# unlikeghost/DeepLearning-MPI

Measured on AMD Instinct MI355X. Metric: images/sec (whole node) ResNet-50 DDP bs=256/GPU, higher is better.
Workload: dtype bf16; 1 GPU; model=resnet50, global_batch=256, image=224, in_channels=3, per_gpu_batch=256, parallelism=dp1, backend=single, device=cuda, optimizer=SGD(momentum=0.9, wd=1e-5), hipgraph=False

## Files before the change

deeplearning_mpi_amd/csrc/binding/conv_bwd.cpp:

```cpp
#include <c10/hip/HIPCachingAllocator.h>

#include <algorithm>
#include <vector>

#include "common.h"
#include "ops.h"

namespace dlmpi_ext {

using dlmpi::ConvArgs;
using dlmpi::ConvPhase;
using dlmpi::DgradStreamArgs;
using dlmpi::make_fastdiv;
using dlmpi::WgradArgs;

c10::optional<at::Tensor> conv2d_dgrad_pro(const at::Tensor& dy, int N, int P, int Q, int K, int lddy, int dyoff,
                                       const at::Tensor& wT, int C, int R, int S, int stride, int pad, int H, int W,
                                       at::Tensor dx, int lddx, int dxoff, const c10::optional<at::Tensor>& res,
                                       int ldres, int resoff, const c10::optional<at::Tensor>& mask, int ldmask,
                                       int maskoff, const c10::optional<at::Tensor>& z, int ldz, int zoff,
                                       const c10::optional<at::Tensor>& z2, int ldz2, int z2off,
                                       const c10::optional<at::Tensor>& mscale,
                                       const c10::optional<at::Tensor>& mshift,
                                       const c10::optional<at::Tensor>& mbits, bool colsum, int pro,
                                       const c10::optional<at::Tensor>& pk0, const c10::optional<at::Tensor>& pk1,
                                       const c10::optional<at::Tensor>& pz, int ldpz, int pzoff,
                                       const c10::optional<at::Tensor>& bias) {
  require_gpu(dy, "dy");
  if (stride > 2) throw std::runtime_error("conv2d_dgrad: stride <= 2 supported");
  if (bias.has_value() && bias->defined() && (bias->scalar_type() != at::kFloat || bias->numel() < C))
    throw std::runtime_error("conv2d_dgrad: bias must be fp32 [C]");
  ConvArgs a{};
  a.f32 = act_f32(dy, "conv2d_dgrad");
  same_type(dy, wT, "conv2d_dgrad wT");
  same_type(dy, dx, "conv2d_dgrad dx");
  same_type(dy, res, "conv2d_dgrad res");
  same_type(dy, mask, "conv2d_dgrad mask");
  same_type(dy, z, "conv2d_dgrad z");
  same_type(dy, z2, "conv2d_dgrad z2");
  a.x = ptr<uint16_t>(dy);
  a.H = P; a.W = Q; a.C = K; a.ldx = lddy; a.xoff = dyoff;
  a.w = ptr<uint16_t>(wT);
  a.ldw = R * S * K;
  a.S = S;
  a.OH = H; a.OW = W;
  a.so = stride; a.sa = 1;
  a.Nimg = N; a.Kout = C;
  fill_epilogue(a, dx, lddx, dxoff, bias, res, ldres, resoff, c10::nullopt, c10::nullopt, false, c10::nullopt);
  a.vec_store = ((lddx % 8) == 0 && (dxoff % 8) == 0) ? 1 : 0;
  a.mask = optr<uint16_t>(mask);
  a.ldmask = ldmask; a.maskoff = maskoff;
  a.z = optr<uint16_t>(z);
  a.ldz = ldz; a.zoff = zoff;
  a.z2 = optr<uint16_t>(z2);
  a.ldz2 = ldz2; a.z2off = z2off;
  a.mscale = optr<float>(mscale);
  a.mshift = optr<float>(mshift);
  a.mbits = optr<uint8_t>(mbits);
  if (a.mbits && (mbits->numel() != (int64_t)N * H * W * (C / 8) || C % 8))
    throw std::runtime_error("conv2d_dgrad: mask bits must be [N*H*W][C/8]");
  a.nstat = a.z2 ? 3 : 2;
  if (a.z && !a.mask && !a.mscale && !a.mbits)
    throw std::runtime_error("conv2d_dgrad: fused BN statistics need the ReLU mask");
  if (a.mscale && (!a.z || !a.mshift)) throw std::runtime_error("conv2d_dgrad: mask from z needs z, scale, shift");
  if ((a.mask || a.mscale || a.mbits) && ((ldmask | maskoff | ldz | zoff | ldz2 | z2off) % 8 != 0 || !a.vec_store))
    throw std::runtime_error("conv2d_dgrad: fused BN tensors must be 8-channel aligned");
  g_ran.dgrad_stream = 0;
  g_ran.conv3 = 0;
  if (R == 1 && S == 1 && K == 8) g_ran.head_dgrad = 0;
  {
    const int mode = a.mscale ? 2 : 0;
    int th, tw, G;
    if (stream3x3_shape(N, H, W, K, C, R, S, stride, pad, pro, a.f32, th, tw, G) && P == H && Q == W && !colsum &&
        !a.mask && !a.mbits && !a.z2 && !a.res && !a.bias && (a.z != nullptr) == (mode == 2) && a.vec_store &&
        a.kvalid == C && (lddy | dyoff) % 8 == 0 && (int64_t)H * W * lddx * 2 < (1ll << 31) &&
        dx.scalar_type() == at::kBFloat16) {
      dlmpi::Conv3StreamArgs c = conv3_args(dy, N, H, W, lddy, dyoff, wT, 1, a.y, lddx, dxoff, th, tw, G);
      c.z = static_cast<const uint16_t*>(a.z);
      c.ldz = ldz; c.zoff = zoff;
      c.mscale = a.mscale; c.mshift = a.mshift;
      c10::optional<at::Tensor> st;
      if (a.z) {
        st = at::empty({(int64_t)G, 2, (int64_t)C}, dy.options().dtype(at::kFloat));
        c.stats = ptr<float>(*st);
      }
      check(dlmpi_conv3x3_stream(&c, mode == 2 ? 2 : 1, cur_stream()), "conv2d_dgrad (stream 3x3)");
      g_ran.conv3 = 1;
      return st;
    }
  }
  {
    const int64_t M = (int64_t)N * H * W;
    const int mode = a.mbits ? 1 : (a.mscale ? 2 : 0);
    int sbm, sbn, G;
    const auto fits = [](int64_t rows, int64_t ld) { return rows * ld < (1ll << 31); };
    if (R == 1 && S == 1 && stride == 1 && pad == 0 && !a.f32 && pro == 0 && !colsum && !a.mask &&
        (a.z != nullptr) == (mode != 0) && a.vec_store && a.kvalid == C && (lddy | dyoff) % 8 == 0 &&
        (!a.res || (ldres | resoff) % 8 == 0) && fits(M, lddy) && fits(M, lddx) && (!a.res || fits(M, ldres)) &&
        (!a.z || fits(M, ldz)) && (!a.z2 || fits(M, ldz2)) && dx.scalar_type() == at::kBFloat16 &&
        dlmpi_dgrad_stream_plan(M, K, C, mode, a.z2 ? 1 : 0, a.res ? 1 : 0, &sbm, &sbn, &G)) {
      DgradStreamArgs sa{};
      sa.x = ptr<uint16_t>(dy);
      sa.ldx = lddy; sa.xoff = dyoff;
      sa.w = ptr<uint16_t>(wT);
      sa.y = reinterpret_cast<uint16_t*>(a.y);
      sa.ldy = lddx; sa.yoff = dxoff;
      sa.y_bytes = (int)std::min<int64_t>(INT32_MAX, (int64_t)dx.numel() * 2);
      sa.M = (int)M; sa.K = K; sa.Kout = C;
      sa.bias = a.bias;
      sa.res = static_cast<const uint16_t*>(a.res);
      sa.ldres = ldres; sa.resoff = resoff;
      sa.z = static_cast<const uint16_t*>(a.z);
      sa.ldz = ldz; sa.zoff = zoff;
      sa.z2 = static_cast<const uint16_t*>(a.z2);
      sa.ldz2 = ldz2; sa.z2off = z2off;
      sa.mbits = a.mbits;
      sa.mscale = a.mscale; sa.mshift = a.mshift;
      sa.G = G; sa.ntiles = C / sbn; sa.mtiles = (int)ceil_div(M, sbm);
      c10::optional<at::Tensor> st;
      if (a.z) {
        st = at::empty({(int64_t)G, (int64_t)a.nstat, (int64_t)C}, dy.options().dtype(at::kFloat));
        sa.stats = ptr<float>(*st);
      }
      check(dlmpi_conv1x1_dgrad_stream(&sa, sbm, sbn, mode, cur_stream()), "conv2d_dgrad (stream 1x1)");
      g_ran.dgrad_stream = 1;
      return st;
    }
  }
  set_kstep(a, K);
  set_prologue(a, pro, pk0, pk1, pz, ldpz, pzoff);
  TileQuery q{(int64_t)N * H * W / (stride * stride), C, (int64_t)R * S * K / (stride * stride), K, R, S, stride, pad,
              H, W, a.f32, pro};
  q.halo_ok = P == H && Q == W;
  q.pipe_ok = g_sw.pipe_dgrad != 0;
  const Tiles t = select_tiles(q);
  int bm = t.bm, bn = t.bn;
  const int pipe = t.pipe;
  const bool halo = t.halo;
  a.ntiles = ceil_div(C, bn);
  a.nphase = stride * stride;
  int tiles = 0;
  for (int ph = 0; ph < stride; ++ph) {
    for (int pw = 0; pw < stride; ++pw) {
      ConvPhase& p = a.ph[ph * stride + pw];
      const int r0 = (ph + pad) % stride, s0 = (pw + pad) % stride;
      p.P = (H - ph + stride - 1) / stride;
      p.Q = (W - pw + stride - 1) / stride;
      p.Tr = r0 < R ? (R - r0 + stride - 1) / stride : 0;
      p.Ts = s0 < S ? (S - s0 + stride - 1) / stride : 0;
      p.dh0 = (ph + pad - r0) / stride; p.dhs = -1;
      p.dw0 = (pw + pad - s0) / stride; p.dws = -1;
      p.wr0 = r0; p.wrs = stride; p.ws0 = s0; p.wss = stride;
      p.oh0 = ph; p.ow0 = pw;
      finish_phase(p, N, K, bm, a.f32);
      p.tile_base = tiles;
      tiles += p.mtiles;
    }
  }
  if (halo) {
    apply_halo(a, N, bm);
    tiles = a.ph[0].mtiles;
// ... 189 lines not shown
  const int bn = a.f32 ? 64 : (w256 ? 256 : 128);
  a.ntiles = ceil_div(a.TC, bn);
  const int tiles = a.mtiles * a.ntiles;
  const int target_blocks = g_sw.wgrad_blocks > 0 ? g_sw.wgrad_blocks : 512;
  const int maxsplit = std::max(1, ceil_div(a.npix, 512));
  int splits = std::max(1, std::min(maxsplit, w256 ? target_blocks / tiles : ceil_div(target_blocks, tiles)));
  int pps = ceil_div(a.npix, splits);
  pps = ceil_div(pps, 64) * 64;
  splits = ceil_div(a.npix, pps);
  a.splits = splits;
  a.pix_per_split = pps;
  a.fdPQ = make_fastdiv((uint32_t)(P * Q));
  a.fdQ = make_fastdiv((uint32_t)Q);
  a.fdC = make_fastdiv((uint32_t)C);
  a.fdS = make_fastdiv((uint32_t)S);
  const int64_t wsz = (int64_t)Ko * a.TC;
  const int G = splits > 1 ? dlmpi_wgrad_reduce_groups(splits, wsz) : 0;
  at::Tensor ws = at::empty({(int64_t)(splits + G) * wsz}, dy.options().dtype(at::kFloat));
  a.ws = ptr<float>(ws);
  check(dlmpi_conv_wgrad(&a, bm, bn, cur_stream()), "conv2d_wgrad");
  wgrad_reduce_or_defer(ws, splits, G, wsz, Ko, R * S, C, Creal, Ko_real, grad);
}

void conv2d_wgrad(const at::Tensor& dy, int lddy, int dyoff, int Ko, const at::Tensor& x, int N, int H, int W, int C,
                  int ldx, int xoff, int R, int S, int stride, int pad, int P, int Q, at::Tensor grad, int Creal,
                  int Ko_real) {
  conv2d_wgrad_pro(dy, lddy, dyoff, Ko, x, N, H, W, C, ldx, xoff, R, S, stride, pad, P, Q, grad, Creal, Ko_real, 0,
                   c10::nullopt, c10::nullopt, 0, 0, 0, c10::nullopt, c10::nullopt);
}

void register_conv_bwd(pybind11::module& m) {
  m.def("conv2d_dgrad", &conv2d_dgrad);
  m.def("conv2d_dgrad_pro", &conv2d_dgrad_pro);
  m.def("conv2d_wgrad", &conv2d_wgrad);
  m.def("conv2d_wgrad_pro", &conv2d_wgrad_pro);
  m.def("set_wgrad_defer", [](bool on) {
    if (!on) wgrad_flush();
    g_wgrad_defer = on;
  });
  m.def("wgrad_flush", &wgrad_flush);
  m.def("wgrad_discard", &wgrad_discard);
  m.def("set_wgrad_batch", [](int n) { g_wgrad_batch = n > 0 && n <= dlmpi::kWgradBatch ? n : dlmpi::kWgradBatch; });
  m.def("set_defer_direct", [](int on) { g_defer_direct = on != 0; });
  m.def("set_wgrad_bypass", [](bool on) { g_wgrad_bypass = on; });
  m.def("wgrad_pending", []() { return (int)g_pending.size(); });
  m.def("wgrad_reduce_launches", []() { return g_reduce_launches; });
  m.def("set_dgrad_stream", [](int mode) { dlmpi_set_dgrad_stream(mode); });
  m.def("set_wgrad_fast", [](int on) { dlmpi_set_wgrad_fast(on); });
  def_int(m, "set_conv_pipe_dgrad", nullptr, &g_sw.pipe_dgrad);
  def_int(m, "set_wgrad3", nullptr, &g_sw.wgrad3);
  def_int(m, nullptr, "wgrad3_last", &g_ran.wgrad3);
  def_int(m, "set_wgrad3_blocks", nullptr, &g_sw.wgrad3_blocks);
  def_int(m, "set_wgrad_blocks", nullptr, &g_sw.wgrad_blocks);
  def_int(m, nullptr, "dgrad_stream_last", &g_ran.dgrad_stream);
  def_int(m, nullptr, "head_dgrad_last", &g_ran.head_dgrad);
}

}
```

deeplearning_mpi_amd/csrc/kernels/conv1x1_dgrad_stream.hip:

```cpp
#include "common.h"

namespace dlmpi {

typedef __attribute__((address_space(3))) void dgs_lds_void;

constexpr int dgs_vmcnt(int n) { return (n & 15) | 0x70 | 0xF00 | ((n >> 4) << 14); }
__device__ __forceinline__ void dgs_barrier() { asm volatile("s_waitcnt lgkmcnt(0)\n\ts_barrier" ::: "memory"); }
__device__ __forceinline__ void dgs_glds(const void* g, char* lds) {
  __builtin_amdgcn_global_load_lds(g, (dgs_lds_void*)lds, 16, 0, 0);
}

template <int BN>
__device__ __forceinline__ int dgs_sw(int r) { return BN == 128 ? (r & 15) : ((r >> 1) & 7); }
template <int BN>
__device__ __forceinline__ int dgs_eoff(int r, int col) {
  return r * (2 * BN) + ((((col >> 3) ^ dgs_sw<BN>(r))) << 4) + ((col & 4) << 1);
}

template <int BM, int BN, int KS, int NW, int WGM, int MASK, bool Z2, bool ADB>
__global__ __launch_bounds__(64 * NW) void conv1x1_dgrad_stream_kernel(const DgradStreamArgs a) {
  constexpr bool Z = MASK != 0;
  static_assert(!Z2 || Z, "z2 needs the fused statistics");
  static_assert(BN == 64 || BN == 128, "tile width");
  constexpr bool RES = !(BN == 64 && BM == 64);
// ... 34 lines not shown
  const int jc = (tid & 7) ^ ((tid >> 3) & 7);
  const int erow = tid / ECH, ej = tid % ECH;
  const char* zp = reinterpret_cast<const char*>(g_zero_page);

  const uint32_t lb = xcd_remap(blockIdx.x, gridDim.x);
  const int nt = lb % a.ntiles, g = lb / a.ntiles;
  const int n0 = nt * BN;
  const bool has_res = RES && a.res != nullptr;

#pragma unroll
  for (int ks = 0; ks < KS; ++ks)
#pragma unroll
    for (int i = 0; i < BL; ++i) {
      const int n = n0 + lrow + RP * i;
      const char* src = (lrow + RP * i < BN && n < a.Kout)
                            ? reinterpret_cast<const char*>(a.w + (int64_t)n * a.K + ks * 64 + 8 * jc) : zp;
      dgs_glds(src, Ws + ks * WROWS * 128 + (RP * i + 8 * wid) * 128);
    }
  auto issue_a = [&](int mt, char* Ab) {
#pragma unroll
    for (int ks = 0; ks < KS; ++ks)
#pragma unroll
      for (int i = 0; i < AL; ++i) {
        const int m = min(mt * BM + lrow + RP * i, a.M - 1);
        dgs_glds(a.x + (uint32_t)(m * a.ldx + a.xoff + ks * 64 + 8 * jc), Ab + ks * BM * 128 + (RP * i + 8 * wid) * 128);
      }
  };
  auto issue_e = [&](int mt, char* Rb, char* Zb, char* Mb) {
#pragma unroll
    for (int i = 0; i < EL; ++i) {
      const int r = erow + EP * i;
      const int m = min(mt * BM + r, a.M - 1);
      const int gj = ej ^ dgs_sw<BN>(r);
      if (has_res)
        dgs_glds(a.res + (uint32_t)(m * a.ldres + a.resoff + n0 + gj * 8), Rb + i * EP * ERB + wid * 1024);
      if constexpr (Z)
        dgs_glds(a.z + (uint32_t)(m * a.ldz + a.zoff + n0 + gj * 8), Zb + i * EP * ERB + wid * 1024);
      if constexpr (Z2)
        dgs_glds(a.z2 + (uint32_t)(m * a.ldz2 + a.z2off + n0 + gj * 8), Zb + (EZ2_OFF - EZ_OFF) + i * EP * ERB + wid * 1024);
    }
    if constexpr (MASK == 1) {
      if (wid < MB_INSTR) {
        const int piece = wid * 64 + lane;
        const int r = piece * MB_PIECE / MBR;
        const int m = min(mt * BM + r, a.M - 1);
        const uint8_t* src = a.mbits + (uint32_t)(m * (a.Kout >> 3) + (n0 >> 3) + (piece * MB_PIECE) % MBR);
        if constexpr (MB_PIECE == 16) __builtin_amdgcn_global_load_lds(src, (dgs_lds_void*)(Mb + wid * 1024), 16, 0, 0);
        else __builtin_amdgcn_global_load_lds(src, (dgs_lds_void*)(Mb + wid * 256), 4, 0, 0);
      }
    }
  };

  const __amdgpu_buffer_rsrc_t yr = __builtin_amdgcn_make_buffer_rsrc(a.y, (short)0, a.y_bytes, 0x00020000);
  f32x4 bq[TN], ms[TN], mh[TN];
#pragma unroll
  for (int ni = 0; ni < TN; ++ni) {
    const int c = n0 + wn * WN + ni * 16 + 4 * fg;
    bq[ni] = a.bias ? *reinterpret_cast<const f32x4*>(a.bias + c) : f32x4{0.f, 0.f, 0.f, 0.f};
    if constexpr (MASK == 2) {
      ms[ni] = *reinterpret_cast<const f32x4*>(a.mscale + c);
      mh[ni] = *reinterpret_cast<const f32x4*>(a.mshift + c);
    }
  }
  float s1[TN][4], s2[TN][4], s3[TN][4];
#pragma unroll
  for (int ni = 0; ni < TN; ++ni)
#pragma unroll
    for (int j = 0; j < 4; ++j) { s1[ni][j] = 0.f; s2[ni][j] = 0.f; s3[ni][j] = 0.f; }
// ... 213 lines not shown
```

deeplearning_mpi_amd/csrc/kernels/dlmpi_kernels.h:

```cpp
#pragma once
#include <hip/hip_runtime_api.h>
#include <stdint.h>

namespace dlmpi {

struct FastDiv {
  uint32_t d, mul, shr;
};
inline FastDiv make_fastdiv(uint32_t d) {
  FastDiv f;
  f.d = d;
  uint32_t l = 0;
  while ((1ull << l) < d) ++l;
  f.mul = (uint32_t)((((1ull << 32) * ((1ull << l) - d)) / d) + 1);
  f.shr = l;
  return f;
}

struct FinArgs {
  int mode;
  double count;
  const float* gamma;
  const float* beta;
  float* running_mean;
// ... 18 lines not shown
  uint16_t* y;
  int ldy, yoff;
  int y_bytes;
  int M, C, Kout;
  const float* bias;
  float* stats;
  int G, ntiles, mtiles;
  int s2, H, W;
  FastDiv fdPQ, fdQ;
  int up2;
  int Cup;
};

struct DgradStreamArgs {
  const uint16_t* x;
  int ldx, xoff;
  const uint16_t* w;
  uint16_t* y;
  int ldy, yoff;
  int y_bytes;
  int M, K, Kout;
  const float* bias;
  const uint16_t* res;
  int ldres, resoff;
  const uint16_t* z;
  int ldz, zoff;
  const uint16_t* z2;
  int ldz2, z2off;
  const uint8_t* mbits;
  const float* mscale;
  const float* mshift;
  float* stats;
  int G, ntiles, mtiles;
};

struct ConvPhase {
  int P, Q;
  int Tr, Ts;
  int dh0, dhs, dw0, dws;
  int wr0, wrs, ws0, wss;
  int oh0, ow0;
  int mtiles;
  int ksteps;
  int tile_base;
  FastDiv fdPQ, fdQ, fdTs;
};

struct ConvArgs {
  const void* x;
  int H, W, C, ldx, xoff;
  const void* w;
  int ldw, S;
  void* y;
  int OH, OW, ldy, yoff;
  int so, sa;
  int out_f32;
  int Nimg, Kout;
  int kvalid;
  int vec_store;
  const float* bias;
  const void* res;
  int ldres, resoff;
  const float* scale;
  const float* shift;
  int relu;
  float* stats;
// ... 267 lines not shown
```

deeplearning_mpi_amd/models/engine.py:

```python
from __future__ import annotations

import contextlib
import os
from typing import NamedTuple, Optional

import torch
import torch.nn as nn

from ..ops.act import Act, Deferred, padc
from ..ops.backend import make_backend
from ..utils.arena import ParamArena
from ..utils.profiler import range as trace_range


@contextlib.contextmanager
def grad_side(be, *tensors):
    side = getattr(be, "side_stream", None)
    if side is None:
        yield
        return
    cur = torch.cuda.current_stream()
    side.wait_stream(cur)
    torch.cuda.set_stream(side)
    try:
# ... 11 lines not shown
def record_on(stream, *objs):
    if _STREAM_HOLD:
        return
    for o in objs:
        if o is None:
            continue
        if isinstance(o, torch.Tensor):
            if o.is_cuda:
                o.record_stream(stream)
        elif isinstance(o, Deferred):
            record_on(stream, *o.bufs())
        elif hasattr(o, "buf") and isinstance(getattr(o, "buf"), torch.Tensor):
            record_on(stream, o.buf)
        elif isinstance(o, (tuple, list)):
            record_on(stream, *o)


_STREAM_HOLD = True

_OUTER_DGRAD = True
_HEAD_DGRAD = True

DEFER_BN_WGRAD = True

DUAL_DGRAD = True
DUAL_MIN_ROWS = 2 * 256 * 28 * 28
DUAL_WGRAD_PRO = True

FUSE_APPLY = True
FUSE_APPLY_MAX_K = 256
FUSE_APPLY_3X3 = True

WGRAD_TAIL_MAIN = True


def img_rows(a, n0: int, n1: int):
    if a is None:
        return None
    if isinstance(a, Deferred):
        return Deferred(a.kind, img_rows(a.src, n0, n1), img_rows(a.z, n0, n1), a.k0, a.k1)
    hw = a.H * a.W
    return Act(a.buf[n0 * hw:n1 * hw], n1 - n0, a.H, a.W, a.C, a.off)


class PendingApply:

    __slots__ = ("y", "z", "scale", "shift", "res", "relu", "mbits", "done")

    def __init__(self, y, z, scale, shift, res, relu, mbits):
        self.y, self.z, self.scale, self.shift, self.res, self.relu, self.mbits = y, z, scale, shift, res, relu, mbits
        self.done = False

    N = property(lambda self: self.y.N)
    H = property(lambda self: self.y.H)
    W = property(lambda self: self.y.W)
    C = property(lambda self: self.y.C)
    device = property(lambda self: self.y.device)

    def resolve(self, be) -> Act:
        if not self.done:
            be.bn_apply(self.z, self.scale, self.shift, self.res, self.relu, self.y, mbits=self.mbits)
            self.done = True
        return self.y


def resolve(be, a):
# ... 171 lines not shown
                if defer_apply == "act":
                    return Deferred.affine(z, scale, shift), ctx
                if defer_apply == "bn":
                    return Deferred.bn(z, scale, shift), ctx
                return z, ctx
            mbits = None
            if save and res is not None and self.relu and self.Kp % 8 == 0:
                mbits = torch.empty(y.rows, self.Kp // 8, dtype=torch.uint8, device=dev)
            if before_res is not None and res is not None:
                before_res()
            ctx = (x, z, y, mean, invstd, scale, shift, res is not None, mbits) if save else None
            if lazy and FUSE_APPLY and out is None:
                return PendingApply(y, z, scale, shift, res, self.relu, mbits), ctx
            be.bn_apply(z, scale, shift, res, self.relu, y, mbits=mbits)
            return y, ctx
        if before_res is not None and res is not None:
            before_res()
        invstd = torch.rsqrt(bn.running_var + bn.eps)
        scale = bn.weight.data * invstd if bn.affine else invstd
        shift = (bn.bias.data if bn.affine else 0.0) - bn.running_mean * scale
        if self.bias is not None:
            shift = shift + self.bias.data * scale
        be.conv_fwd(x, wf, self.Kp, self.R, self.S, self.stride, self.pad, y, res=res, scale=scale.contiguous(),
                    shift=shift.contiguous(), relu=self.relu)
        return y, None

    @staticmethod
    def fuse_spec(ctx, z2=None) -> BwdFuse:
        x, z, y, mean, invstd, scale, shift, has_res, mbits = ctx
        if has_res or z2 is not None:
            return BwdFuse(None if mbits is not None else y, z, z2, mbits=mbits)
        return BwdFuse(None, z, None, scale, shift)

    def bwd(self, be, ctx, dy: Act, need_dx=True, dx_res: Act = None, dyr_out: Act = None, ymask: Act = None,
            use_own_mask=True, pre=None, k2=1, fuse_next=None, colsum=False, before_res=None, dx_out: Act = None):
        ar = self.arena
        bn = self.bn
        dg_in, dg_w, dg_b = None, None, None
        if bn is not None and need_dx and pre is not None and dyr_out is None and self.dual:
            x, z = ctx[0], ctx[1]
            if (z.off == z.C and z.ld == 2 * z.C and dy.off == 0 and dy.ld == z.ld
                    and dy.buf.data_ptr() == z.buf.data_ptr()):
                mean, invstd = ctx[3], ctx[4]
                gam = bn.weight.data if bn.affine else None
                dzd = be.bn_bwd_deferred(dy, z, mean, invstd, gam, ar.grad_flat(bn.weight) if bn.affine else None,
                                         ar.grad_flat(bn.bias) if bn.affine else None, pre=pre, k2=k2)
                with grad_side(be, *bufs(dzd, x)):
                    if bn.affine:
                        ar.ready(bn.weight, bn.bias)
                    if self.bias is not None:
                        ar.ready(self.bias)
                    self._wgrad(be, dzd if (DUAL_WGRAD_PRO and getattr(be, "prologue", False)) else be.materialize(dzd), x)
                    ar.ready(self.conv.weight)
                dg_w, dg_b = be.dual_weights(ar.get_compute(self.h_dg), self.Cp, self.Kp, dzd.k0)
                dg_in = Act(z.buf, z.N, z.H, z.W, 2 * z.C)
                bn = None
        if dg_in is not None:
            x = ctx[0]
        elif bn is not None:
            x, z, y, mean, invstd = ctx[:5]
            if pre is not None:
                mask = None
            else:
                mask = ymask if ymask is not None else (y if (self.relu and use_own_mask) else None)
            gam = bn.weight.data if bn.affine else None
            dgam = ar.grad_flat(bn.weight) if bn.affine else None
            dbet = ar.grad_flat(bn.bias) if bn.affine else None
            defer = not need_dx and DEFER_BN_WGRAD and getattr(be, "prologue", False)
# ... 10 lines not shown
                    if self.bias is not None:
                        ar.ready(self.bias)
                    ar.ready(self.conv.weight)
            else:
                with grad_side(be, *bufs(dz, x)):
                    if bn.affine:
                        ar.ready(bn.weight, bn.bias)
                    if self.bias is not None:
                        ar.ready(self.bias)
                    self._wgrad(be, dz, x)
                    ar.ready(self.conv.weight)
        else:
            x, y = ctx
            assert not self.relu, "ReLU without BN is not used by the engine models"
            dz = dy
            with grad_side(be, *bufs(dz, x)):
                if self.bias is not None:
                    if self.Kp == self.K:
                        be.channel_sum(dz, ar.grad_flat(self.bias))
                    else:
                        tmp = torch.empty(self.Kp, dtype=be.dt, device=dz.device)
                        be.fill_(tmp, 0.0)
                        be.channel_sum(dz, tmp)
                        if getattr(self, "_kidx", None) is None or self._kidx.device != dz.device:
                            self._kidx = torch.arange(self.K, device=dz.device)
                        be.gather_(ar.grad_flat(self.bias), tmp, self._kidx, accumulate=True)
                    ar.ready(self.bias)
                self._wgrad(be, dz, x)
                ar.ready(self.conv.weight)
        if not need_dx:
            return None
        if before_res is not None:
            before_res()
        if dx_out is not None:
            assert (dx_out.N, dx_out.H, dx_out.W, dx_out.C) == (x.N, x.H, x.W, self.Cp), (dx_out, x, self.Cp)
            dx = dx_out
        else:
            dx = Act.empty(x.N, x.H, x.W, self.Cp, be.act_dtype, x.device)
        if dg_in is not None:
            part = be.conv_dgrad(dg_in, dg_w, self.Cp, 1, 1, 1, 0, dx, res=dx_res, fuse=fuse_next, colsum=colsum,
                                 bias=dg_b)
            return (dx, part) if (fuse_next is not None or colsum) else dx
        if (self.K == 1 and self.R == 1 and self.S == 1 and self.stride == 1 and dx_res is None and not colsum
                and fuse_next is not None and fuse_next.scale is not None and fuse_next.z2 is None
                and hasattr(be, "outer_dgrad_bn") and _OUTER_DGRAD):
            part = be.outer_dgrad_bn(be.materialize(dz), ar.get_compute(self.h_dg), self.Kp, dx, fuse_next)
            return dx, part
        if (2 <= self.K <= 4 and self.R == 1 and self.S == 1 and self.stride == 1 and dx_res is None and not colsum
                and fuse_next is not None and fuse_next.scale is not None and fuse_next.z2 is None
                and hasattr(be, "head_dgrad_bn") and _HEAD_DGRAD):
            part = be.head_dgrad_bn(be.materialize(dz), self.K, ar.get_compute(self.h_dg), self.Kp, dx, fuse_next)
            return dx, part
        part = be.conv_dgrad(dz, ar.get_compute(self.h_dg), self.Cp, self.R, self.S, self.stride, self.pad, dx,
                             res=dx_res, fuse=fuse_next, colsum=colsum)
        return (dx, part) if (fuse_next is not None or colsum) else dx


class S2DConvUnit(ConvUnit):

    CS = 4

    def __init__(self, arena: ParamArena, conv, bn=None, relu=True):
        w = conv.weight
        K, Cin, R, S = w.shape
        assert conv.stride == (2, 2) and conv.padding[0] == conv.padding[1] and conv.groups == 1
        assert Cin <= self.CS and conv.dilation == (1, 1)
        self.arena, self.conv, self.bn, self.relu = arena, conv, bn, relu
        self.linear = False
        self.K, self.Cin, self.R0, self.S0, self.pad0 = K, Cin, R, S, conv.padding[0]
        self.R, self.S = (R + 1) // 2, (S + 1) // 2
        self.stride, self.pad = 1, 0
        self.Cp = 4 * self.CS
        self.Kp = padc(K)
        self.bias = conv.bias
        self._bias_pad = None
        self.h_dg = None
        self.h_slots = []
        for vh in (0, 1):
            for vw in (0, 1):
                v = w.data[:, :, vh::2, vw::2]
                self.h_slots.append(arena.add_compute(v, (self.Kp, self.R, self.S, self.CS),
                                                      (K, v.shape[2], v.shape[3], Cin), (0, 2, 3, 1)))
        self.w2 = None
        self._w2idx = None
        arena.post_refresh.append(self._build_w2)
        self._gidx = None

# ... 212 lines not shown
```

deeplearning_mpi_amd/models/resnet.py:

```python
from __future__ import annotations


import torch
import torch.nn as nn
import torch.nn.functional as F

from ..ops.act import Act, padc
from .engine import PendingApply, BwdFuse, ConvUnit, EngineModule, S2DConvUnit, record_on, resolve


def conv3x3(i, o, stride=1):
    return nn.Conv2d(i, o, 3, stride, 1, bias=False)


def conv1x1(i, o, stride=1):
    return nn.Conv2d(i, o, 1, stride, 0, bias=False)


class BasicBlock(nn.Module):
    expansion = 1

    def __init__(self, inplanes, planes, stride=1, downsample=None):
        super().__init__()
        self.conv1 = conv3x3(inplanes, planes, stride)
# ... 85 lines not shown
            ctxs.append(first[1])
        for u in self.u[1 if first is not None else 0:-1]:
            h, c = u.fwd(be, h, train, save=save, lazy=lazy)
            ctxs.append(c)
        join = None
        if br is not None:
            def join():
                main.wait_stream(br)
                record_on(main, idn, cd)
            if not _LATE_JOIN:
                join()
                join = None
        elif self.ud is not None:
            idn, cd = self.ud.fwd(be, x, train, save=save, defer_apply=ds_defer)
        else:
            idn, cd = resolve(be, x), None
        y, c = self.u[-1].fwd(be, h, train, res=idn, save=save, before_res=join, lazy=lazy)
        ctxs.append(c)
        return y, (ctxs, cd)

    def fuse_spec(self, st):
        ctxs, cd = st
        return ConvUnit.fuse_spec(ctxs[-1], z2=cd[1] if cd is not None else None)

    def out_slot(self, st):
        return self.u[-1].dy_slot(st[0][-1])

    def bwd(self, be, st, dy: Act, pre=None, fuse_prev=None, fuse_inner=False, dx_out=None):
        ctxs, cd = st
        slot = lambda k: self.u[k].dy_slot(ctxs[k])
        ylast = ctxs[-1][2]
        n = len(self.u)
        spec = lambda k: ConvUnit.fuse_spec(ctxs[k])
        if pre is not None:
            br = getattr(be, "branch_stream", None) if self.ud is not None else None
            if br is not None:
                main = torch.cuda.current_stream()
                br.wait_stream(main)
                with torch.cuda.stream(br):
                    dres = self.ud.bwd(be, cd, dy, pre=pre, k2=2)
                record_on(br, dy, pre)
            dh, part = self.u[-1].bwd(be, ctxs[-1], dy, pre=pre, k2=1, fuse_next=spec(n - 2), dx_out=slot(n - 2))
            for k in range(n - 2, 0, -1):
                dh, part = self.u[k].bwd(be, ctxs[k], dh, pre=part, fuse_next=spec(k - 1), dx_out=slot(k - 1))
            join = None
            if br is not None:
                def join():
                    main.wait_stream(br)
                    record_on(main, dres)
                if not _LATE_JOIN:
                    join()
                    join = None
            elif self.ud is not None:
                dres = self.ud.bwd(be, cd, dy, pre=pre, k2=2)
            else:
                dres = dy
            return self.u[0].bwd(be, ctxs[0], dh, dx_res=dres, pre=part, fuse_next=fuse_prev, before_res=join,
                                 dx_out=dx_out)
        inner = fuse_inner or any(c[2] is None for c in ctxs[:-1])
        if self.ud is None:
            dyr = Act.empty(dy.N, dy.H, dy.W, dy.C, be.act_dtype, dy.device)
            dh = self.u[-1].bwd(be, ctxs[-1], dy, dyr_out=dyr, fuse_next=spec(n - 2) if inner else None,
                                dx_out=slot(n - 2))
        else:
            dyr = None
            dh = self.u[-1].bwd(be, ctxs[-1], dy, fuse_next=spec(n - 2) if inner else None, dx_out=slot(n - 2))
        part = None
        if inner:
            dh, part = dh
        for k in range(n - 2, 0, -1):
            if inner:
                dh, part = self.u[k].bwd(be, ctxs[k], dh, pre=part, fuse_next=spec(k - 1), dx_out=slot(k - 1))
            else:
                dh = self.u[k].bwd(be, ctxs[k], dh, dx_out=slot(k - 1))
        if self.ud is not None:
            dres = self.ud.bwd(be, cd, dy, ymask=ylast)
        else:
            dres = dyr
        out = self.u[0].bwd(be, ctxs[0], dh, dx_res=dres, pre=part, fuse_next=fuse_prev, dx_out=dx_out)
        return out


class ResNet(EngineModule):
    def __init__(self, block, layers, num_classes=1000, in_channels=3):
        super().__init__()
        self.inplanes = 64
        self.in_channels = in_channels
        self.conv1 = nn.Conv2d(in_channels, 64, kernel_size=7, stride=2, padding=3, bias=False)
        self.bn1 = nn.BatchNorm2d(64)
        self.relu = nn.ReLU(inplace=True)
        self.maxpool = nn.MaxPool2d(kernel_size=3, stride=2, padding=1)
        self.layer1 = self._make_layer(block, 64, layers[0])
        self.layer2 = self._make_layer(block, 128, layers[1], stride=2)
        self.layer3 = self._make_layer(block, 256, layers[2], stride=2)
        self.layer4 = self._make_layer(block, 512, layers[3], stride=2)
        self.avgpool = nn.AdaptiveAvgPool2d((1, 1))
        self.fc = nn.Linear(512 * block.expansion, num_classes)
        for m in self.modules():
            if isinstance(m, nn.Conv2d):
                nn.init.kaiming_normal_(m.weight, mode="fan_out", nonlinearity="relu")
            elif isinstance(m, nn.BatchNorm2d):
                nn.init.constant_(m.weight, 1)
                nn.init.constant_(m.bias, 0)

    def _make_layer(self, block, planes, blocks, stride=1):
        downsample = None
        if stride != 1 or self.inplanes != planes * block.expansion:
            downsample = nn.Sequential(conv1x1(self.inplanes, planes * block.expansion, stride),
                                       nn.BatchNorm2d(planes * block.expansion))
# ... 113 lines not shown
```

deeplearning_mpi_amd/ops/backend.py:

```python
from __future__ import annotations

import os
import weakref
import struct

import torch
import torch.nn.functional as F

from .act import Act, Deferred


_AUX_STREAMS = {}
_BACKENDS = weakref.WeakSet()


def _new_aux_stream(idx, C, role):
    with torch.cuda.device(idx):
        st = torch.cuda.ExternalStream(C.create_stream(), device=torch.device("cuda", idx))
        C.set_aux_stream(st.cuda_stream, role)
    return st


def _aux_stream(device, C, role):
    idx = device.index if device.index is not None else torch.cuda.current_device()
# ... 126 lines not shown
    def conv_fwd_bn_apply(self, xp, w, K, z: Act, bias, stats, count, gamma, beta, rm, rv, momentum, eps, scale,
                          shift, save_mean, save_invstd):
        x, res = xp.z, xp.res
        rs = rh = None
        if isinstance(res, Deferred):
            assert res.kind == "bn", res
            res, rs, rh = res.src, res.k0, res.k1
        y = xp.y
        self.C.conv2d_fwd_bn_apply(x.buf, x.N, x.H, x.W, x.C, x.ld, x.off, w, K, z.buf, z.ld, z.off, bias, stats,
                                   xp.scale, xp.shift, res.buf, res.ld, res.off, rs, rh, y.buf, y.ld, y.off, xp.mbits,
                                   float(count), gamma, beta, rm, rv, float(momentum), float(eps), scale, shift,
                                   save_mean, save_invstd)

    def conv3_pro_ok(self, z: Act, y: Act) -> bool:
        return bool(self.C.conv3_pro_ok(z.N, z.H, z.W, z.C, 64, z.ld, z.off, y.ld, y.off, y.ld, y.off))

    def conv3_fwd_bn_apply(self, xp, w, K, z: Act, bias, stats, count, gamma, beta, rm, rv, momentum, eps, scale,
                           shift, save_mean, save_invstd):
        x, y = xp.z, xp.y
        r = self.C.conv3x3_fwd_bn_apply(x.buf, x.N, x.H, x.W, x.ld, x.off, w, z.buf, z.ld, z.off, bias, stats,
                                        xp.scale, xp.shift, y.buf, y.ld, y.off, float(count), gamma, beta, rm, rv,
                                        float(momentum), float(eps), scale, shift, save_mean, save_invstd)
        if r < 0:
            self.bn_apply(xp.z, xp.scale, xp.shift, None, True, y)
            self.conv_fwd_bn(y, w, K, 3, 3, 1, 1, z, bias, stats, count, gamma, beta, rm, rv, momentum, eps, scale,
                             shift, save_mean, save_invstd)

    def conv_fwd_bnbwd(self, x: Act, w, K, R, S, stride, pad, y: Act, fuse):
        z = fuse.z
        return self.C.conv2d_fwd_bnbwd(x.buf, x.N, x.H, x.W, x.C, x.ld, x.off, w, K, R, S, stride, pad, y.buf, y.ld,
                                       y.off, z.buf, z.ld, z.off, fuse.scale, fuse.shift)

    def conv_dgrad(self, dy: Act, wT, C, R, S, stride, pad, dx: Act, res: Act = None, fuse=None, colsum=False,
                   bias=None):
        m, z, z2, sc, sh, mb = fuse if fuse is not None else (None, None, None, None, None, None)

        def t(a):
            return (a.buf, a.ld, a.off) if a is not None else (None, 0, 0)

        dy = self.materialize(dy)
        return self.C.conv2d_dgrad_pro(dy.buf, dy.N, dy.H, dy.W, dy.C, dy.ld, dy.off, wT, C, R, S, stride, pad, dx.H,
                                       dx.W, dx.buf, dx.ld, dx.off, *t(res), *t(m), *t(z), *t(z2), sc, sh, mb,
                                       bool(colsum and fuse is None), 0, None, None, None, 0, 0, bias)

    def dual_weights(self, wT, C, K, coef):
        w2 = torch.empty(C, 2 * K, dtype=self.act_dtype, device=self.device)
        b = torch.empty(C, dtype=torch.float32, device=self.device)
        self.C.dual_dgrad_weights(wT, C, K, coef, w2, b)
        return w2, b

    def convT_fwd(self, x: Act, wf, Cout, y: Act, bias=None):
        self.C.convT2x2_fwd(x.buf, x.N, x.H, x.W, x.C, x.ld, x.off, wf, Cout, y.buf, y.ld, y.off, bias)

    def wgrad_defer(self, on: bool):
        self.C.set_wgrad_defer(bool(on))

    def wgrad_flush(self):
        self.C.wgrad_flush()

    def wgrad_discard(self):
        self.C.wgrad_discard()

    def wgrad_bypass(self, on: bool):
        self.C.set_wgrad_bypass(bool(on))

    def conv_wgrad(self, dy, x, R, S, stride, pad, grad, Creal, Ko_real):
        direct = R == 1 and S == 1 and stride == 1 and pad == 0
        if isinstance(dy, Deferred) and isinstance(x, Deferred) or (isinstance(x, Deferred) and not direct):
            x = self.materialize(x)
        dy, pa, ca, _, zb, zld, zoff = self._pro(dy)
        x, pb, sb, hb, _, _, _ = self._pro(x)
        assert pa in (0, 2) and pb in (0, 1)
        self.C.conv2d_wgrad_pro(dy.buf, dy.ld, dy.off, dy.C, x.buf, x.N, x.H, x.W, x.C, x.ld, x.off, R, S, stride,
                                pad, dy.H, dy.W, grad, Creal, Ko_real, pa, ca, zb, zld, zoff, pb, sb, hb)

    def bn_finalize(self, stats, ntiles, C, count, gamma, beta, rm, rv, momentum, eps, scale, shift, save_mean,
# ... 253 lines not shown
    def conv_mtiles(self, N, H, W, C, K, R, S, stride, pad, pro=False):
        return 1

    def conv_fwd(self, x, w, K, R, S, stride, pad, y: Act, bias=None, res=None, scale=None, shift=None,
                 relu=False, stats=None, kvalid=0):
        x = self.materialize(x)
        wk = w.view(K, R, S, x.C).permute(0, 3, 1, 2).to(self.dt)
        out = F.conv2d(x.nchw().to(self.dt), wk, None, stride, pad)
        if bias is not None:
            out = out + bias.view(1, -1, 1, 1)
        if stats is not None:
            stats.view(-1, 2, K)[0, 0].copy_(out.sum((0, 2, 3)))
            stats.view(-1, 2, K)[0, 1].copy_((out * out).sum((0, 2, 3)))
        if scale is not None:
            out = out * scale.view(1, -1, 1, 1) + shift.view(1, -1, 1, 1)
        if res is not None:
            out = out + res.nchw().to(self.dt)
        if relu:
            out = F.relu(out)
        self._store(y, out)

    def conv_fwd_bn(self, x, w, K, R, S, stride, pad, z: Act, bias, stats, count, gamma, beta, rm, rv, momentum,
                    eps, scale, shift, save_mean, save_invstd):
        self.conv_fwd(x, w, K, R, S, stride, pad, z, bias=bias, stats=stats)
        self.bn_finalize(stats, stats.shape[0], K, count, gamma, beta, rm, rv, momentum, eps, scale, shift,
                         save_mean, save_invstd)

    def dual_weights(self, wT, C, K, coef):
        w = wT.reshape(C, K).to(self.dt)
        c = coef.to(self.dt)
        w2 = torch.cat([w * c[0], w * c[1]], 1).to(self.act_dtype)
        return w2, (w * c[2]).sum(1)

    def conv_dgrad(self, dy, wT, C, R, S, stride, pad, dx: Act, res=None, fuse=None, colsum=False, bias=None):
        dy = self.materialize(dy)
        K = dy.C
        wk = wT.view(C, R, S, K).permute(3, 0, 1, 2).to(self.dt)
        g = torch.nn.grad.conv2d_input((dx.N, C, dx.H, dx.W), wk, dy.nchw().to(self.dt), stride, pad)
        if bias is not None:
            g = g + bias.to(self.dt).view(1, -1, 1, 1)
        if res is not None:
            g = g + res.nchw().to(self.dt)
        if fuse is None:
            self._store(dx, g)
            if colsum:
                v = dx.nhwc().to(self.dt)
                return torch.stack([v.sum((0, 1, 2)), (v * v).sum((0, 1, 2))]).unsqueeze(0)
            return None
        m, z, z2, sc, sh, mb = fuse
        if mb is not None:
            g = g * self._unpack_bits(mb, z).permute(0, 3, 1, 2)
        elif m is not None:
            g = g * (m.nchw() > 0)
        else:
            keep = (z.nhwc().to(self.dt) * sc + sh) > 0
            g = g * keep.permute(0, 3, 1, 2)
        self._store(dx, g)
        v = dx.nhwc().to(self.dt)
        rows = [v.sum((0, 1, 2)), (v * z.nhwc().to(self.dt)).sum((0, 1, 2))]
        if z2 is not None:
            rows.append((v * z2.nhwc().to(self.dt)).sum((0, 1, 2)))
        return torch.stack(rows).unsqueeze(0)

    def conv_fwd_bn_apply(self, xp, w, K, z: Act, bias, stats, *fin):
        self.bn_apply(xp.z, xp.scale, xp.shift, xp.res, xp.relu, xp.y, mbits=xp.mbits)
        self.conv_fwd_bn(xp.y, w, K, 1, 1, 1, 0, z, bias, stats, *fin)

    def conv3_fwd_bn_apply(self, xp, w, K, z: Act, bias, stats, *fin):
        self.bn_apply(xp.z, xp.scale, xp.shift, None, True, xp.y)
        self.conv_fwd_bn(xp.y, w, K, 3, 3, 1, 1, z, bias, stats, *fin)

    def conv_fwd_bnbwd(self, x: Act, w, K, R, S, stride, pad, y: Act, fuse):
        wk = w.view(K, R, S, x.C).permute(0, 3, 1, 2).to(self.dt)
        out = F.conv2d(x.nchw().to(self.dt), wk, None, stride, pad)
# ... 325 lines not shown
```

Measured before the change: 13450 images/sec.

## Compute stride-2 downsample dgrad at compact resolution and scatter via residual read

The 1x1 stride-2 downsample convolution's data gradient is now computed only at the subsampled positions (N×H/2×W/2) rather than writing a full-resolution gradient that is zero at three of every four positions. The main branch's streaming 1x1 dgrad kernel reads this compact residual, mapping each output row to its subsampled source with fast division and loading zeros at odd positions. This removes the write and re-read of a mostly-zero full-size tensor and the work of producing it. It adds per-row index arithmetic in the kernel's residual load, a new eligibility check, and a hard error if the streaming path cannot be used.

```diff
diff --git a/deeplearning_mpi_amd/csrc/binding/conv_bwd.cpp b/deeplearning_mpi_amd/csrc/binding/conv_bwd.cpp
--- a/deeplearning_mpi_amd/csrc/binding/conv_bwd.cpp
+++ b/deeplearning_mpi_amd/csrc/binding/conv_bwd.cpp
@@ -13,6 +13,24 @@
 using dlmpi::DgradStreamArgs;
 using dlmpi::make_fastdiv;
 using dlmpi::WgradArgs;
+
+static bool dgs_operands_ok(int64_t M, int lddy, int dyoff, int lddx, int dxoff, bool has_res, int64_t Mres,
+                            int ldres, int resoff, bool has_z, int ldz, int zoff, bool has_z2, int ldz2, int z2off) {
+  const auto fits = [](int64_t rows, int64_t ld) { return rows * ld < (1ll << 31); };
+  return (lddy | dyoff | lddx | dxoff) % 8 == 0 && fits(M, lddy) && fits(M, lddx) &&
+         (!has_res || ((ldres | resoff) % 8 == 0 && fits(Mres, ldres))) &&
+         (!has_z || ((ldz | zoff) % 8 == 0 && fits(M, ldz))) && (!has_z2 || ((ldz2 | z2off) % 8 == 0 && fits(M, ldz2)));
+}
+
+bool dgrad_res_sub_ok(int N, int H, int W, int K, int C, int P, int Q, int mode, bool z2, bool f32, int lddy,
+                      int dyoff, int lddx, int dxoff, int ldres, int resoff, int ldz, int zoff, int ldz2, int z2off) {
+  int bm, bn, G;
+  const int64_t M = (int64_t)N * H * W;
+  return !f32 && N > 0 && P > 0 && Q > 0 && H == 2 * P && W == 2 * Q && C % 8 == 0 && ldres >= C &&
+         dgs_operands_ok(M, lddy, dyoff, lddx, dxoff, true, (int64_t)N * P * Q, ldres, resoff, mode != 0, ldz, zoff,
+                         z2, ldz2, z2off) &&
+         dlmpi_dgrad_stream_plan(M, K, C, mode, z2 ? 1 : 0, 1, &bm, &bn, &G) != 0;
+}
 
 c10::optional<at::Tensor> conv2d_dgrad_pro(const at::Tensor& dy, int N, int P, int Q, int K, int lddy, int dyoff,
                                        const at::Tensor& wT, int C, int R, int S, int stride, int pad, int H, int W,
@@ -25,9 +43,13 @@
                                        const c10::optional<at::Tensor>& mbits, bool colsum, int pro,
                                        const c10::optional<at::Tensor>& pk0, const c10::optional<at::Tensor>& pk1,
                                        const c10::optional<at::Tensor>& pz, int ldpz, int pzoff,
-                                       const c10::optional<at::Tensor>& bias) {
+                                       const c10::optional<at::Tensor>& bias, int res_sub = 0) {
   require_gpu(dy, "dy");
   if (stride > 2) throw std::runtime_error("conv2d_dgrad: stride <= 2 supported");
+  if (res_sub != 0 && res_sub != 2) throw std::runtime_error("conv2d_dgrad: res_sub is 0 or 2");
+  if (!(res.has_value() && res->defined())) res_sub = 0;
+  if (res_sub && res->numel() < ((int64_t)N * (H / 2) * (W / 2) - 1) * ldres + resoff + C)
+    throw std::runtime_error("conv2d_dgrad: compact residual smaller than [N][H/2][W/2][ldres]");
   if (bias.has_value() && bias->defined() && (bias->scalar_type() != at::kFloat || bias->numel() < C))
     throw std::runtime_error("conv2d_dgrad: bias must be fp32 [C]");
   ConvArgs a{};
@@ -93,11 +115,12 @@
     const int64_t M = (int64_t)N * H * W;
     const int mode = a.mbits ? 1 : (a.mscale ? 2 : 0);
     int sbm, sbn, G;
-    const auto fits = [](int64_t rows, int64_t ld) { return rows * ld < (1ll << 31); };
-    if (R == 1 && S == 1 && stride == 1 && pad == 0 && !a.f32 && pro == 0 && !colsum && !a.mask &&
-        (a.z != nullptr) == (mode != 0) && a.vec_store && a.kvalid == C && (lddy | dyoff) % 8 == 0 &&
-        (!a.res || (ldres | resoff) % 8 == 0) && fits(M, lddy) && fits(M, lddx) && (!a.res || fits(M, ldres)) &&
-        (!a.z || fits(M, ldz)) && (!a.z2 || fits(M, ldz2)) && dx.scalar_type() == at::kBFloat16 &&
+    const bool sub_ok = !res_sub || (H % 2 == 0 && W % 2 == 0);
+    if (R == 1 && S == 1 && stride == 1 && pad == 0 && !a.f32 && pro == 0 && !colsum && !a.mask && sub_ok &&
+        (a.z != nullptr) == (mode != 0) && a.vec_store && a.kvalid == C &&
+        dgs_operands_ok(M, lddy, dyoff, lddx, dxoff, a.res != nullptr, res_sub ? M / 4 : M, ldres, resoff,
+                        a.z != nullptr, ldz, zoff, a.z2 != nullptr, ldz2, z2off) &&
+        dx.scalar_type() == at::kBFloat16 &&
         dlmpi_dgrad_stream_plan(M, K, C, mode, a.z2 ? 1 : 0, a.res ? 1 : 0, &sbm, &sbn, &G)) {
       DgradStreamArgs sa{};
       sa.x = ptr<uint16_t>(dy);
@@ -110,6 +133,11 @@
       sa.bias = a.bias;
       sa.res = static_cast<const uint16_t*>(a.res);
       sa.ldres = ldres; sa.resoff = resoff;
+      if (res_sub) {
+        sa.res_sub = res_sub; sa.P = H / 2; sa.Q = W / 2;
+        sa.fdHW = make_fastdiv((uint32_t)(H * W));
+        sa.fdW = make_fastdiv((uint32_t)W);
+      }
       sa.z = static_cast<const uint16_t*>(a.z);
       sa.ldz = ldz; sa.zoff = zoff;
       sa.z2 = static_cast<const uint16_t*>(a.z2);
@@ -127,6 +155,8 @@
       return st;
     }
   }
+  if (res_sub)
+    throw std::runtime_error("conv2d_dgrad: res_sub needs the streaming 1x1 data gradient (dgrad_res_sub_ok)");
   set_kstep(a, K);
   set_prologue(a, pro, pk0, pk1, pz, ldpz, pzoff);
   TileQuery q{(int64_t)N * H * W / (stride * stride), C, (int64_t)R * S * K / (stride * stride), K, R, S, stride, pad,
@@ -382,6 +412,22 @@
 void register_conv_bwd(pybind11::module& m) {
   m.def("conv2d_dgrad", &conv2d_dgrad);
   m.def("conv2d_dgrad_pro", &conv2d_dgrad_pro);
+  m.def("conv2d_dgrad_pro", [](const at::Tensor& dy, int N, int P, int Q, int K, int lddy, int dyoff,
+                               const at::Tensor& wT, int C, int R, int S, int stride, int pad, int H, int W,
+                               at::Tensor dx, int lddx, int dxoff, const c10::optional<at::Tensor>& res, int ldres,
+                               int resoff, const c10::optional<at::Tensor>& mask, int ldmask, int maskoff,
+                               const c10::optional<at::Tensor>& z, int ldz, int zoff,
+                               const c10::optional<at::Tensor>& z2, int ldz2, int z2off,
+                               const c10::optional<at::Tensor>& mscale, const c10::optional<at::Tensor>& mshift,
+                               const c10::optional<at::Tensor>& mbits, bool colsum, int pro,
+                               const c10::optional<at::Tensor>& pk0, const c10::optional<at::Tensor>& pk1,
+                               const c10::optional<at::Tensor>& pz, int ldpz, int pzoff,
+                               const c10::optional<at::Tensor>& bias) {
+    return conv2d_dgrad_pro(dy, N, P, Q, K, lddy, dyoff, wT, C, R, S, stride, pad, H, W, dx, lddx, dxoff, res, ldres,
+                            resoff, mask, ldmask, maskoff, z, ldz, zoff, z2, ldz2, z2off, mscale, mshift, mbits, colsum,
+                            pro, pk0, pk1, pz, ldpz, pzoff, bias, 0);
+  });
+  m.def("dgrad_res_sub_ok", &dgrad_res_sub_ok);
   m.def("conv2d_wgrad", &conv2d_wgrad);
   m.def("conv2d_wgrad_pro", &conv2d_wgrad_pro);
   m.def("set_wgrad_defer", [](bool on) {
diff --git a/deeplearning_mpi_amd/csrc/kernels/conv1x1_dgrad_stream.hip b/deeplearning_mpi_amd/csrc/kernels/conv1x1_dgrad_stream.hip
--- a/deeplearning_mpi_amd/csrc/kernels/conv1x1_dgrad_stream.hip
+++ b/deeplearning_mpi_amd/csrc/kernels/conv1x1_dgrad_stream.hip
@@ -90,8 +90,18 @@
       const int r = erow + EP * i;
       const int m = min(mt * BM + r, a.M - 1);
       const int gj = ej ^ dgs_sw<BN>(r);
-      if (has_res)
-        dgs_glds(a.res + (uint32_t)(m * a.ldres + a.resoff + n0 + gj * 8), Rb + i * EP * ERB + wid * 1024);
+      if (has_res) {
+        int rr = m;
+        bool hit = true;
+        if (a.res_sub) {
+          const uint32_t n = fdiv((uint32_t)m, a.fdHW), rem = (uint32_t)m - n * a.fdHW.d;
+          const uint32_t h = fdiv(rem, a.fdW), w = rem - h * a.fdW.d;
+          hit = ((h | w) & 1u) == 0;
+          rr = (int)((n * a.P + (h >> 1)) * a.Q + (w >> 1));
+        }
+        const uint16_t* src = a.res + (uint32_t)(rr * a.ldres + a.resoff + n0 + gj * 8);
+        dgs_glds(hit ? reinterpret_cast<const char*>(src) : zp, Rb + i * EP * ERB + wid * 1024);
+      }
       if constexpr (Z)
         dgs_glds(a.z + (uint32_t)(m * a.ldz + a.zoff + n0 + gj * 8), Zb + i * EP * ERB + wid * 1024);
       if constexpr (Z2)
diff --git a/deeplearning_mpi_amd/csrc/kernels/dlmpi_kernels.h b/deeplearning_mpi_amd/csrc/kernels/dlmpi_kernels.h
--- a/deeplearning_mpi_amd/csrc/kernels/dlmpi_kernels.h
+++ b/deeplearning_mpi_amd/csrc/kernels/dlmpi_kernels.h
@@ -74,6 +74,8 @@
   const float* mshift;
   float* stats;
   int G, ntiles, mtiles;
+  int res_sub, P, Q;
+  FastDiv fdHW, fdW;
 };
 
 struct ConvPhase {
diff --git a/deeplearning_mpi_amd/models/engine.py b/deeplearning_mpi_amd/models/engine.py
--- a/deeplearning_mpi_amd/models/engine.py
+++ b/deeplearning_mpi_amd/models/engine.py
@@ -67,6 +67,13 @@
 FUSE_APPLY_3X3 = True
 
 WGRAD_TAIL_MAIN = True
+
+COMPACT_DS_DGRAD = True
+
+
+class SubRes(NamedTuple):
+    act: Act
+    sub: int
 
 
 def img_rows(a, n0: int, n1: int):
@@ -304,8 +311,19 @@
             return BwdFuse(None if mbits is not None else y, z, z2, mbits=mbits)
         return BwdFuse(None, z, None, scale, shift)
 
+    def takes_sub_res(self, be, ctx, dual: bool, fuse_next, dx_out: Optional[Act]) -> bool:
+        ok = getattr(be, "dgrad_res_sub_ok", None)
+        if (not COMPACT_DS_DGRAD or ok is None or self.linear or self.R != 1 or self.S != 1 or self.stride != 1
+                or self.pad != 0):
+            return False
+        x = ctx[0]
+        K = 2 * self.Kp if dual else self.Kp
+        lddx, dxoff = (dx_out.ld, dx_out.off) if dx_out is not None else (self.Cp, 0)
+        return bool(ok(x.N, x.H, x.W, K, self.Cp, K, lddx, dxoff, self.Cp, fuse_next))
+
     def bwd(self, be, ctx, dy: Act, need_dx=True, dx_res: Act = None, dyr_out: Act = None, ymask: Act = None,
-            use_own_mask=True, pre=None, k2=1, fuse_next=None, colsum=False, before_res=None, dx_out: Act = None):
+            use_own_mask=True, pre=None, k2=1, fuse_next=None, colsum=False, before_res=None, dx_out: Act = None,
+            compact_dx=False):
         ar = self.arena
         bn = self.bn
         dg_in, dg_w, dg_b = None, None, None
@@ -382,6 +400,17 @@
             return None
         if before_res is not None:
             before_res()
+        res_sub = 0
+        if isinstance(dx_res, SubRes):
+            dx_res, res_sub = dx_res
+        if compact_dx:
+            assert (self.R, self.S, self.stride, self.pad) == (1, 1, 2, 0) and dg_in is None, self.conv
+            assert dx_res is None and fuse_next is None and not colsum and dx_out is None
+            dz = be.materialize(dz)
+            assert (x.H, x.W) == (2 * dz.H, 2 * dz.W), (x, dz)
+            dxc = Act.empty(x.N, dz.H, dz.W, self.Cp, be.act_dtype, x.device)
+            be.conv_dgrad(dz, ar.get_compute(self.h_dg), self.Cp, 1, 1, 1, 0, dxc)
+            return SubRes(dxc, 2)
         if dx_out is not None:
             assert (dx_out.N, dx_out.H, dx_out.W, dx_out.C) == (x.N, x.H, x.W, self.Cp), (dx_out, x, self.Cp)
             dx = dx_out
@@ -389,7 +418,7 @@
             dx = Act.empty(x.N, x.H, x.W, self.Cp, be.act_dtype, x.device)
         if dg_in is not None:
             part = be.conv_dgrad(dg_in, dg_w, self.Cp, 1, 1, 1, 0, dx, res=dx_res, fuse=fuse_next, colsum=colsum,
-                                 bias=dg_b)
+                                 bias=dg_b, res_sub=res_sub)
             return (dx, part) if (fuse_next is not None or colsum) else dx
         if (self.K == 1 and self.R == 1 and self.S == 1 and self.stride == 1 and dx_res is None and not colsum
                 and fuse_next is not None and fuse_next.scale is not None and fuse_next.z2 is None
@@ -402,7 +431,7 @@
             part = be.head_dgrad_bn(be.materialize(dz), self.K, ar.get_compute(self.h_dg), self.Kp, dx, fuse_next)
             return dx, part
         part = be.conv_dgrad(dz, ar.get_compute(self.h_dg), self.Cp, self.R, self.S, self.stride, self.pad, dx,
-                             res=dx_res, fuse=fuse_next, colsum=colsum)
+                             res=dx_res, fuse=fuse_next, colsum=colsum, res_sub=res_sub)
         return (dx, part) if (fuse_next is not None or colsum) else dx
 
 
diff --git a/deeplearning_mpi_amd/models/resnet.py b/deeplearning_mpi_amd/models/resnet.py
--- a/deeplearning_mpi_amd/models/resnet.py
+++ b/deeplearning_mpi_amd/models/resnet.py
@@ -141,13 +141,22 @@
         ylast = ctxs[-1][2]
         n = len(self.u)
         spec = lambda k: ConvUnit.fuse_spec(ctxs[k])
+
+        def compact(fused):
+            ud, u0 = self.ud, self.u[0]
+            if ud is None or (ud.R, ud.S, ud.stride, ud.pad) != (1, 1, 2, 0) or ud.bn is None:
+                return False
+            dual = fused and u0.bn is not None and slot(0) is not None
+            return u0.takes_sub_res(be, ctxs[0], dual, fuse_prev, dx_out)
+
         if pre is not None:
             br = getattr(be, "branch_stream", None) if self.ud is not None else None
+            cdx = compact(True)
             if br is not None:
                 main = torch.cuda.current_stream()
                 br.wait_stream(main)
                 with torch.cuda.stream(br):
-                    dres = self.ud.bwd(be, cd, dy, pre=pre, k2=2)
+                    dres = self.ud.bwd(be, cd, dy, pre=pre, k2=2, compact_dx=cdx)
                 record_on(br, dy, pre)
             dh, part = self.u[-1].bwd(be, ctxs[-1], dy, pre=pre, k2=1, fuse_next=spec(n - 2), dx_out=slot(n - 2))
             for k in range(n - 2, 0, -1):
@@ -161,7 +170,7 @@
                     join()
                     join = None
             elif self.ud is not None:
-                dres = self.ud.bwd(be, cd, dy, pre=pre, k2=2)
+                dres = self.ud.bwd(be, cd, dy, pre=pre, k2=2, compact_dx=cdx)
             else:
                 dres = dy
             return self.u[0].bwd(be, ctxs[0], dh, dx_res=dres, pre=part, fuse_next=fuse_prev, before_res=join,
@@ -183,7 +192,7 @@
             else:
                 dh = self.u[k].bwd(be, ctxs[k], dh, dx_out=slot(k - 1))
         if self.ud is not None:
-            dres = self.ud.bwd(be, cd, dy, ymask=ylast)
+            dres = self.ud.bwd(be, cd, dy, ymask=ylast, compact_dx=compact(inner))
         else:
             dres = dyr
         out = self.u[0].bwd(be, ctxs[0], dh, dx_res=dres, pre=part, fuse_next=fuse_prev, dx_out=dx_out)
diff --git a/deeplearning_mpi_amd/ops/backend.py b/deeplearning_mpi_amd/ops/backend.py
--- a/deeplearning_mpi_amd/ops/backend.py
+++ b/deeplearning_mpi_amd/ops/backend.py
@@ -182,7 +182,7 @@
                                        y.off, z.buf, z.ld, z.off, fuse.scale, fuse.shift)
 
     def conv_dgrad(self, dy: Act, wT, C, R, S, stride, pad, dx: Act, res: Act = None, fuse=None, colsum=False,
-                   bias=None):
+                   bias=None, res_sub=0):
         m, z, z2, sc, sh, mb = fuse if fuse is not None else (None, None, None, None, None, None)
 
         def t(a):
@@ -191,7 +191,19 @@
         dy = self.materialize(dy)
         return self.C.conv2d_dgrad_pro(dy.buf, dy.N, dy.H, dy.W, dy.C, dy.ld, dy.off, wT, C, R, S, stride, pad, dx.H,
                                        dx.W, dx.buf, dx.ld, dx.off, *t(res), *t(m), *t(z), *t(z2), sc, sh, mb,
-                                       bool(colsum and fuse is None), 0, None, None, None, 0, 0, bias)
+                                       bool(colsum and fuse is None), 0, None, None, None, 0, 0, bias, int(res_sub))
+
+    def dgrad_res_sub_ok(self, N, H, W, K, C, lddy, lddx, dxoff, ldres, fuse=None) -> bool:
+        m, z, z2, sc, sh, mb = fuse if fuse is not None else (None, None, None, None, None, None)
+        if m is not None:
+            return False
+        mode = 1 if mb is not None else (2 if sc is not None else 0)
+        if (z is not None) != (mode != 0):
+            return False
+        return bool(self.C.dgrad_res_sub_ok(N, H, W, K, C, H // 2, W // 2, mode, z2 is not None, self.f32, lddy, 0,
+                                            lddx, dxoff, ldres, 0, z.ld if z is not None else 0,
+                                            z.off if z is not None else 0, z2.ld if z2 is not None else 0,
+                                            z2.off if z2 is not None else 0))
 
     def dual_weights(self, wT, C, K, coef):
         w2 = torch.empty(C, 2 * K, dtype=self.act_dtype, device=self.device)
@@ -511,14 +523,22 @@
         w2 = torch.cat([w * c[0], w * c[1]], 1).to(self.act_dtype)
         return w2, (w * c[2]).sum(1)
 
-    def conv_dgrad(self, dy, wT, C, R, S, stride, pad, dx: Act, res=None, fuse=None, colsum=False, bias=None):
+    def dgrad_res_sub_ok(self, N, H, W, K, C, lddy, lddx, dxoff, ldres, fuse=None) -> bool:
+        return H % 2 == 0 and W % 2 == 0
+
+    def conv_dgrad(self, dy, wT, C, R, S, stride, pad, dx: Act, res=None, fuse=None, colsum=False, bias=None,
+                   res_sub=0):
         dy = self.materialize(dy)
         K = dy.C
         wk = wT.view(C, R, S, K).permute(3, 0, 1, 2).to(self.dt)
         g = torch.nn.grad.conv2d_input((dx.N, C, dx.H, dx.W), wk, dy.nchw().to(self.dt), stride, pad)
         if bias is not None:
             g = g + bias.to(self.dt).view(1, -1, 1, 1)
-        if res is not None:
+        if res is not None and res_sub:
+            assert res_sub == 2 and (dx.H, dx.W) == (2 * res.H, 2 * res.W), (res_sub, dx, res)
+            g = g.clone()
+            g[:, :, ::2, ::2] += res.nchw().to(self.dt)
+        elif res is not None:
             g = g + res.nchw().to(self.dt)
         if fuse is None:
             self._store(dx, g)
```

Measured after the change: 13510 images/sec, median of 6. Within noise of the previous version (+0.4%).
